# k-sheridan/ekf_vio

Hardware: AMD Instinct MI355X
Metric: filter steps/sec (predict+update) (higher is better)
Workload: dtype f32

## Files before the change

ekf_vio_amd/csrc/chol_persist.inc:

```

#ifndef PERSIST_POLL_SLEEP_LAZY
#define PERSIST_POLL_SLEEP_LAZY 12
#endif
#ifndef PERSIST_POLL_SLEEP
#define PERSIST_POLL_SLEEP 2
#endif

struct PollBound {
    int spin_limit, wait_ticks;
};
struct PersistArgs {
    float* S;
    int lds;
    float* L;
    int ldl;
    float* Linv;
    int mb, idb0;
    int* info;
    unsigned long long* Lsign;
    int* ready;
    int* fin;
    int* abort_flag;
    long long* dbg;
    PersistGrid grid;
// ... 245 lines not shown
        float yq = 0.f, rd = 0.f, ro = 0.f;
        if (sq >= 0) {
            yq = ga.zrow[cq] - ga.mu[sq];
            rd = ga.Rm[2 * cq];
            ro = ga.Rm[2 * (cq ^ 1) + 1];
        }
        tab[tid] = yq, tab[64 + tid] = rd, tab[128 + tid] = ro;
    }
    auto column_flags = [&](int kb, const int* zflag) -> PollLane {
        const int ax = alo + tid - 2;
        return {tid == 0 ? a.pan + iy * mb + kb : tid == 1 ? zflag : (tid >= 2 && ax <= ahi) ? a.pan + (mb + ax) * mb + kb : nullptr, 1};
    };
    float kv[16], w2[16];
    {
        float wv[16];
        const int scl = max(sq, 0);
#pragma unroll
        for (int ps = 0; ps < 16; ps++) wv[ps] = ga.P[(size_t)min(ib * PB + wave + 4 * ps, ga.n - 1) * ga.ld + scl];
#pragma unroll
        for (int ps = 0; ps < 16; ps++) asm volatile("" : "+v"(wv[ps]));
#pragma unroll
        for (int ps = 0; ps < 16; ps++) Th[(wave + 4 * ps) * 65 + lane] = (sq >= 0 && ib * PB + wave + 4 * ps < ga.n) ? wv[ps] : 0.f;
        __syncthreads();
#pragma unroll
        for (int q = 0; q < 16; q++) {
            kv[q] = 0.f;
            w2[q] = Th[r * 65 + mma64_col(wc, lane, q)];
        }
    }
    auto fetch = [&](int kb) -> unsigned long long {
        const bool gk = kb >= cb;
        float hv[16];
        unsigned long long neg;
        if constexpr (WAIT) {
            persist_wait(a, column_flags(kb, gk ? a.pan + iz * mb + kb : nullptr), tid, kb < mb - 2);
            load_tile_sc1(Ti, bL, (unsigned)(kb * PB) * (unsigned)ldl + (unsigned)(iy * PB), ldl, tid);
            if (gk) load_tile_sc1(Tj, bL, (unsigned)(kb * PB) * (unsigned)ldl + (unsigned)(iz * PB), ldl, tid);
#pragma unroll
            for (int ps = 0; ps < 16; ps++)
                hv[ps] = __builtin_bit_cast(float, __builtin_amdgcn_raw_buffer_load_b32(bL, ((unsigned)(kb * PB + wave + 4 * ps) * (unsigned)ldl + (unsigned)(mb * PB) + sqc) * 4u, 0, 16));
#pragma unroll
            for (int ps = 0; ps < 16; ps++) hv[ps] = (sq >= 0) ? hv[ps] : 0.f;
#pragma unroll
            for (int ps = 0; ps < 16; ps++) Th[(wave + 4 * ps) * PLD + lane] = hv[ps];
            neg = ld_sign_sc1(a.Lsign + kb);
        } else {
            load_tile(Ti, a.L + (size_t)kb * PB * ldl + (size_t)iy * PB, ldl, tid);
            if (gk) load_tile(Tj, a.L + (size_t)kb * PB * ldl + (size_t)iz * PB, ldl, tid);
#pragma unroll
            for (int ps = 0; ps < 16; ps++) hv[ps] = a.L[(size_t)(kb * PB + wave + 4 * ps) * ldl + (size_t)(mb * PB) + sqc];
#pragma unroll
            for (int ps = 0; ps < 16; ps++) hv[ps] = (sq >= 0) ? hv[ps] : 0.f;
#pragma unroll
            for (int ps = 0; ps < 16; ps++) Th[(wave + 4 * ps) * PLD + lane] = hv[ps];
            neg = a.Lsign[kb];
        }
        return neg;
    };
    auto products = [&](int kb, unsigned long long neg, bool z_unsigned) {
        if (kb >= cb) {
            const f32x16 up = (z_unsigned && neg != 0ull) ? mma64_signed(Ti, 1, PLD, Tj, 1, PLD, wr, wc, lane, neg) : mma64(Ti, 1, PLD, Tj, 1, PLD, wr, wc, lane);
#pragma unroll
            for (int q = 0; q < 16; q++) kv[q] = kv[q] + up[q];
        }
        if (alo <= ahi) {
            f32x16 up;
            if constexpr (WAIT) {
                up = (neg == 0ull) ? mma64(Ti, 1, PLD, Th, 1, PLD, wr, wc, lane) : mma64_signed(Ti, 1, PLD, Th, 1, PLD, wr, wc, lane, neg);
            } else {
                if (__builtin_amdgcn_readfirstlane((int)(neg != 0ull))) {
                    __syncthreads();
                    sign_cols(Ti, Ti, neg, tid);
                    __syncthreads();
                }
                up = mma64(Ti, 1, PLD, Th, 1, PLD, wr, wc, lane);
            }
#pragma unroll
            for (int q = 0; q < 16; q++) w2[q] = w2[q] - up[q];
        }
        if (WAIT && a.dbg && tid == 0 && mb <= 8 && (ib == 0 || ib == 6) && (cb == 0 || cb == 3 || cb == 7))
            a.dbg[100 + 8 * ((ib ? 3 : 0) + (cb == 0 ? 0 : cb == 3 ? 1 : 2)) + kb] = (long long)__builtin_amdgcn_s_memrealtime();
    };
    if constexpr (WAIT) {
        for (int kb = 0; kb < mb - 2; kb++) {
            __syncthreads();
            const unsigned long long neg = fetch(kb);
            __syncthreads();
            products(kb, neg, false);
        }
    } else {
        for (int kb = 0; kb < mb; kb++) {
            __syncthreads();
            const unsigned long long neg = fetch(kb);
            __syncthreads();
            products(kb, neg, false);
        }
    }
    if constexpr (WAIT) {
        const int kl = mb - 1, k6 = mb - 2;
        const bool gk6 = k6 >= cb;
        const __amdgpu_buffer_rsrc_t bI = persist_rsrc(a.Linv, (unsigned)(mb * PB * PB));
        const bool zi = a.grid.compact() && cb == kl;
        __syncthreads();
        persist_wait(a, column_flags(k6, gk6 ? a.pan + iz * mb + k6 : (zi ? nullptr : a.fin + iz * mb + kl)), tid, false);
        RegTile ql, qi, qj;
        float hq[16];
        unsigned long long neg6;
        {
            RegTile pi6, pj6;
            float h6[16];
            pi6.request(bL, (unsigned)(k6 * PB) * (unsigned)ldl + (unsigned)(iy * PB), ldl, tid);
            if (gk6) pj6.request(bL, (unsigned)(k6 * PB) * (unsigned)ldl + (unsigned)(iz * PB), ldl, tid);
#pragma unroll
            for (int ps = 0; ps < 16; ps++)
                h6[ps] = __builtin_bit_cast(float, __builtin_amdgcn_raw_buffer_load_b32(bL, ((unsigned)(k6 * PB + wave + 4 * ps) * (unsigned)ldl + (unsigned)(mb * PB) + sqc) * 4u, 0, 16));
            neg6 = ld_sign_sc1(a.Lsign + k6);
            pi6.put(Ti, tid);
            if (gk6) pj6.put(Tj, tid);
#pragma unroll
            for (int ps = 0; ps < 16; ps++) Th[(wave + 4 * ps) * PLD + lane] = (sq >= 0) ? h6[ps] : 0.f;
        }
        persist_wait(a, a.ready + kl, nullptr, nullptr, tid, 4, false);
        ql.request(bL, (unsigned)(kl * PB) * (unsigned)ldl + (unsigned)(kl * PB), ldl, tid);
        qi.request(bS, (unsigned)(kl * PB) * (unsigned)a.lds + (unsigned)(iy * PB), a.lds, tid);
        if (!zi) qj.request(bS, (unsigned)(kl * PB) * (unsigned)a.lds + (unsigned)(iz * PB), a.lds, tid);
        const float4 qv = ld_sc1(bI, (unsigned)(kl * PB * PB) + tid * 4);
        const unsigned long long neg7 = ld_sign_sc1(a.Lsign + kl);
#pragma unroll
        for (int ps = 0; ps < 16; ps++)
            hq[ps] = __builtin_bit_cast(float, __builtin_amdgcn_raw_buffer_load_b32(bS, ((unsigned)(kl * PB + wave + 4 * ps) * (unsigned)a.lds + (unsigned)(mb * PB) + sqc) * 4u, 0, 16));
        products(mb - 2, neg6, false);
        __syncthreads();
        ql.put(Tl, tid);
        qi.put(Ti, tid);
        if (zi) identity_tile(Tj, tid);
        else qj.put(Tj, tid);
        inv_put(qv, Tinv, tid);
#pragma unroll
        for (int ps = 0; ps < 16; ps++) Th[(wave + 4 * ps) * PLD + lane] = (sq >= 0) ? hq[ps] : 0.f;
        __syncthreads();
        float* const t3[3] = {Ti, Tj, Th};
        tri_solve_fwd_n<3>(t3, Tl, Tinv, wave, lane);
        __syncthreads();
        products(kl, neg7, true);
    }
#pragma unroll
    for (int q = 0; q < 16; q++) kv[q] = (fabsf(kv[q]) > EKF_FLUSH_THRESH) ? kv[q] : 0.f;
    float* Kt = a.K + (size_t)(cb * PB) * a.ldk + (size_t)ib * PB;
    float* Gt = ga.G + (size_t)(cb * PB) * ga.ld + (size_t)ib * PB;
    float acc = 0.f;
#pragma unroll
    for (int q = 0; q < 16; q++) {
        const int c = mma64_col(wc, lane, q), cg = cb * PB + c;
        Kt[(size_t)c * a.ldk + r] = kv[q];
        float g = 0.f;
        if (cg < m) {
            const float x = kv[q] * tab[64 + c], y = kv[q ^ 1] * tab[128 + c];
            const float kr = ((cg ^ 1) < cg) ? (y + x) : (x + y);
            g = kr - w2[q];
            acc = acc + kv[q] * tab[c];
        }
        Gt[(size_t)c * ga.ld + r] = g;
    }
    __syncthreads();
    float* part = Th;
    part[(wc * 2 + (lane >> 5)) * 64 + r] = acc;
    __syncthreads();
    if (tid < 64) ga.Wt[(size_t)cb * ga.ld + (size_t)ib * PB + tid] = ((part[tid] + part[64 + tid]) + part[128 + tid]) + part[192 + tid];
}

template <bool WAIT>
__device__ __forceinline__ void t2_tile(const PersistArgs& a, float* Ti, float* Tj, float* Tl, float* Tinv, int ta, int tb, int tid, long long* dbg = nullptr) {
    const int lane = tid & 63, wave = tid >> 6, wr = wave & 1, wc = wave >> 1;
    const int r = wr * 32 + (lane & 31);
    const int mb = a.mb, ldl = a.ldl;
    const bool diag = ta == tb;
    const __amdgpu_buffer_rsrc_t bL = persist_rsrc(a.L, (unsigned)ldl * (unsigned)(mb * PB));
    float tab[16], tba[16];
    {
        const float* sab = a.Sg + (size_t)tb * PB * a.ldsg + (size_t)ta * PB;
        const float* sba = a.Sg + (size_t)ta * PB * a.ldsg + (size_t)tb * PB;
#pragma unroll
        for (int q = 0; q < 16; q++) {
            const int c = mma64_col(wc, lane, q);
            tab[q] = sab[(size_t)c * a.ldsg + r];
            tba[q] = diag ? 0.f : sba[(size_t)c * a.ldsg + r];
        }
    }
    const int ia = mb + ta, ib = mb + tb;
    auto apply = [&](int kb, unsigned long long neg) {
        const float* Bj = diag ? Ti : Tj;
        f32x16 up;
        if constexpr (WAIT) {
            up = (neg == 0ull) ? mma64(Ti, 1, PLD, Bj, 1, PLD, wr, wc, lane) : mma64_signed(Ti, 1, PLD, Bj, 1, PLD, wr, wc, lane, neg);
        } else if (__builtin_amdgcn_readfirstlane((int)(neg != 0ull))) {
            sign_cols(Tl, Ti, neg, tid);
            __syncthreads();
            up = mma64(Tl, 1, PLD, Bj, 1, PLD, wr, wc, lane);
            __syncthreads();
        } else {
            up = mma64(Ti, 1, PLD, Bj, 1, PLD, wr, wc, lane);
        }
#pragma unroll
        for (int q = 0; q < 16; q++) tab[q] = tab[q] - up[q];
        if (!diag) {
#pragma unroll
            for (int q = 0; q < 16; q++) Tl[r * PLD + mma64_col(wc, lane, q)] = up[q];
            __syncthreads();
#pragma unroll
            for (int q = 0; q < 16; q++) tba[q] = tba[q] - Tl[mma64_col(wc, lane, q) * PLD + r];
        }
        if (dbg && tid == 0) dbg[kb] = (long long)__builtin_amdgcn_s_memrealtime();
    };
    if constexpr (WAIT) {
        for (int kb = 0; kb < mb - 2; kb++) {
            __syncthreads();
            persist_wait(a, nullptr, a.pan + ia * mb + kb, diag ? nullptr : a.pan + ib * mb + kb, tid, 1, true);
            load_tile_sc1(Ti, bL, (unsigned)(kb * PB) * (unsigned)ldl + (unsigned)(ia * PB), ldl, tid);
            if (!diag) load_tile_sc1(Tj, bL, (unsigned)(kb * PB) * (unsigned)ldl + (unsigned)(ib * PB), ldl, tid);
            const unsigned long long neg = ld_sign_sc1(a.Lsign + kb);
            __syncthreads();
            apply(kb, neg);
        }
    } else {
        for (int kb = 0; kb < mb; kb++) {
            __syncthreads();
            load_tile(Ti, a.L + (size_t)kb * PB * ldl + (size_t)ia * PB, ldl, tid);
            if (!diag) load_tile(Tj, a.L + (size_t)kb * PB * ldl + (size_t)ib * PB, ldl, tid);
            const unsigned long long neg = a.Lsign[kb];
            __syncthreads();
            apply(kb, neg);
        }
    }
    if constexpr (WAIT) {
        const int kl = mb - 1, k6 = mb - 2;
        const __amdgpu_buffer_rsrc_t bS = persist_rsrc(a.S, (unsigned)a.lds * (unsigned)(mb * PB));
        const __amdgpu_buffer_rsrc_t bI = persist_rsrc(a.Linv, (unsigned)(mb * PB * PB));
        __syncthreads();
        persist_wait(a, a.ready + kl, a.pan + ia * mb + k6, diag ? nullptr : a.pan + ib * mb + k6, tid, 4, false);
        RegTile pi6, pj6, ql, qi, qj;
        pi6.request(bL, (unsigned)(k6 * PB) * (unsigned)ldl + (unsigned)(ia * PB), ldl, tid);
        if (!diag) pj6.request(bL, (unsigned)(k6 * PB) * (unsigned)ldl + (unsigned)(ib * PB), ldl, tid);
        const unsigned long long neg6 = ld_sign_sc1(a.Lsign + k6);
        ql.request(bL, (unsigned)(kl * PB) * (unsigned)ldl + (unsigned)(kl * PB), ldl, tid);
        qi.request(bS, (unsigned)(kl * PB) * (unsigned)a.lds + (unsigned)(ia * PB), a.lds, tid);
        if (!diag) qj.request(bS, (unsigned)(kl * PB) * (unsigned)a.lds + (unsigned)(ib * PB), a.lds, tid);
        const float4 qv = ld_sc1(bI, (unsigned)(kl * PB * PB) + tid * 4);
        const unsigned long long neg7 = ld_sign_sc1(a.Lsign + kl);
        pi6.put(Ti, tid);
        if (!diag) pj6.put(Tj, tid);
        __syncthreads();
        apply(k6, neg6);
        __syncthreads();
        ql.put(Tl, tid);
        qi.put(Ti, tid);
        if (!diag) qj.put(Tj, tid);
        inv_put(qv, Tinv, tid);
        __syncthreads();
        if (diag) tri_solve_fwd(Ti, Tl, Tinv, wave, lane);
        else tri_solve_fwd2(Ti, Tj, Tl, Tinv, wave, lane);
        __syncthreads();
        apply(kl, neg7);
    }
    __syncthreads();
#pragma unroll
    for (int q = 0; q < 16; q++) {
        const int c = mma64_col(wc, lane, q);
        Ti[c * PLD + r] = (ta * PB + r < a.nstate && tb * PB + c < a.nstate) ? tab[q] : 0.f;
        if (!diag) Tj[c * PLD + r] = (tb * PB + r < a.nstate && ta * PB + c < a.nstate) ? tba[q] : 0.f;
    }
    __syncthreads();
    store_tile(Ti, a.T2 + (size_t)tb * PB * a.ldt + (size_t)ta * PB, a.ldt, tid);
    if (!diag) store_tile(Tj, a.T2 + (size_t)ta * PB * a.ldt + (size_t)tb * PB, a.ldt, tid);
    if (dbg && tid == 0) dbg[15] = (long long)__builtin_amdgcn_s_memrealtime();
}

template <bool SC1>
__device__ __forceinline__ float persist_ldf(const float* p) {
    if constexpr (SC1) return __hip_atomic_load(p, __ATOMIC_RELAXED, __HIP_MEMORY_SCOPE_AGENT);
    else return *p;
}
template <bool SC1>
__device__ __forceinline__ void persist_tile_x(f32x4 (&x)[4], const float* G, int ld, int wave, int lane) {
    const int li = lane & 15, g = lane >> 4;
#pragma unroll
    for (int b = 0; b < 4; b++)
#pragma unroll
        for (int v = 0; v < 4; v++) x[b][v] = persist_ldf<SC1>(G + (size_t)(16 * b + 4 * g + v) * ld + 16 * wave + li);
}
__device__ __forceinline__ void persist_diag_block(float* D, const float* P, int tr, int tc, int lane, unsigned long long neg) {
    const int li = lane & 15, lk = lane >> 4;
    const int rb = 16 * tr, cb = 16 * tc;
    const float* ap = P + rb + li + lk * PLD;
    const float* bp = P + cb + li + lk * PLD;
    f32x4 u = {0.f, 0.f, 0.f, 0.f};
    if (neg == 0ull) {
#pragma unroll
        for (int q = 0; q < PB; q += 4) u = __builtin_amdgcn_mfma_f32_16x16x4f32(bp[q * PLD], ap[q * PLD], u, 0, 0, 0);
    } else {
#pragma unroll 4
        for (int q = 0; q < PB; q += 4) {
            float av = ap[q * PLD];
            if ((neg >> (q + lk)) & 1ull) av = -av;
            u = __builtin_amdgcn_mfma_f32_16x16x4f32(bp[q * PLD], av, u, 0, 0, 0);
        }
    }
    float t[4];
#pragma unroll
    for (int gq = 0; gq < 4; gq++) t[gq] = D[(cb + 4 * lk + gq) * PLD + rb + li];
#pragma unroll
    for (int gq = 0; gq < 4; gq++) D[(cb + 4 * lk + gq) * PLD + rb + li] = t[gq] - u[gq];
}


struct GTile {
    int ia[16];
    int ib;
    float v[16], rd[16], ro[16];
};
__device__ __forceinline__ void gtile_idx(GTile& t, const GatherArgs& ga, int m, int rb, int cb, int mb, int idb0, int tid) {
    if (rb < mb) {
        const int c = cb * PB + (tid & 63);
        t.ib = (c < m) ? ga.idx[c] : 0;
#pragma unroll
        for (int ps = 0; ps < 16; ps++) {
            const int rc = max(min(rb * PB + (tid >> 6) + 4 * ps, m - 1), 0);
            t.ia[ps] = max(ga.idx[rc], 0);
            t.rd[ps] = ga.Rm[2 * rc];
            t.ro[ps] = ga.Rm[2 * rc + 1];
        }
    } else if (rb < idb0) {
#pragma unroll
        for (int ps = 0; ps < 16; ps++) {
            const int c = cb * PB + (tid >> 6) + 4 * ps;
            t.ia[ps] = (c < m) ? ga.idx[c] : 0;
        }
// ... 274 lines not shown
        PEXIT();
    }

    if (role.kind == ROLE_LEAD || role.kind == ROLE_LEAD_GATHER0) {
        if (!compact) gather_body<false>(ga, ga.nb1 + role.n, persist_dyn_lds);
        else if (role.kind == ROLE_LEAD_GATHER0) {
            const int cb = role.a;
            const int m = ga.m_dev ? *ga.m_dev : ga.m;
            GTile t;
            gtile_idx(t, ga, m, 1, cb, mb, a.idb0, tid);
            gtile_pin(t);
            gtile_val(t, ga, m, 1, cb, mb, a.idb0, tid);
            gtile_pinv(t);
            gtile_put(t, Tl, ga, m, 1, cb, mb, a.idb0, tid);
            __syncthreads();
            store_tile_sc1<false>(Tl, bS, (unsigned)(cb * PB) * (unsigned)lds + (unsigned)PB, lds, tid);
            persist_publish(a.fin + 1 * mb + cb, tid);
        }
        if (a.gain) {
            const int tb = role.n;
            __syncthreads();
            if (role.a < a.idb0 - mb) {
                if (a.t2) gain_tile2<true>(a, ga, Ti, Tj, Tl, Tinv, persist_dyn_lds, persist_dyn_lds + PB * PLD, role.a, role.b, tid);
                else gain_tile(a, Ti, Tj, Tl, Tinv, role.a, role.b, tid);
                if (a.dbg && tid == 0 && tb < 104) a.dbg[200 + tb] = (long long)__builtin_amdgcn_s_memrealtime();
            }
        }
        PEXIT();
    }
    const int idb0 = a.idb0;
    if (role.kind == ROLE_GATHER0) {
        const int cb = role.a;
        const int m = ga.m_dev ? *ga.m_dev : ga.m;
        GTile t;
        gtile_idx(t, ga, m, 1, cb, mb, idb0, tid);
        gtile_pin(t);
        gtile_val(t, ga, m, 1, cb, mb, idb0, tid);
        gtile_pinv(t);
        gtile_put(t, Tl, ga, m, 1, cb, mb, idb0, tid);
        __syncthreads();
        store_tile_sc1<false>(Tl, bS, (unsigned)(cb * PB) * (unsigned)lds + (unsigned)PB, lds, tid);
        persist_publish(a.fin + 1 * mb + cb, tid);
        PEXIT();
    }
    const int i = role.a, j = role.b, hidx = role.n;
    const int k0 = (i >= idb0) ? (i - idb0) : 0;
    const int klast = (i == j) ? j - 2 : j - 1;
    const unsigned oij = (unsigned)(j * PB) * (unsigned)lds + (unsigned)(i * PB);
    float tv[16];
    if (fused) {
        const int m = ga.m_dev ? *ga.m_dev : ga.m;
        const bool step0 = k0 == 0 && klast >= 0;
        GTile tn, ti_, tj_;
        gtile_idx(tn, ga, m, i, j, mb, idb0, tid);
        if (step0) {
            gtile_idx(ti_, ga, m, i, 0, mb, idb0, tid);
            if (i != j) gtile_idx(tj_, ga, m, j, 0, mb, idb0, tid);
        }
        gtile_pin(tn);
        if (step0) gtile_pin(ti_);
        gtile_val(tn, ga, m, i, j, mb, idb0, tid);
        if (step0) {
            gtile_val(ti_, ga, m, i, 0, mb, idb0, tid);
            if (i != j) gtile_val(tj_, ga, m, j, 0, mb, idb0, tid);
        }
        gtile_pinv(tn);
        gtile_put(tn, Tl, ga, m, i, j, mb, idb0, tid);
        if (step0) {
            gtile_put(ti_, Ti, ga, m, i, 0, mb, idb0, tid);
            if (i != j) gtile_put(tj_, Tj, ga, m, j, 0, mb, idb0, tid);
        }
        __syncthreads();
#pragma unroll
        for (int q = 0; q < 16; q++) tv[q] = Tl[mma64_col(wc, lane, q) * PLD + r];
        __syncthreads();
    } else {
#pragma unroll
        for (int q = 0; q < 16; q++) tv[q] = S[oij + (size_t)mma64_col(wc, lane, q) * lds + r];
    }
#define HSTAMP(n)                                                                                                       \
    do {                                                                                                                \
        if (a.dbg && i == j + 1 && i < mb && k == klast && tid == 0) a.dbg[600 + 8 * j + (n)] = (long long)__builtin_amdgcn_s_memtime(); \
    } while (0)
    unsigned long long neg = 0ull;
    int k = k0;
    for (; k <= klast; k++) {
        HSTAMP(0);
        const bool lazy = !(k == klast && i <= j + 1);
        const bool early = a.early_sources && k >= 1;
        const bool src_ident = compact && k >= 1 && i >= idb0 && i - idb0 == k;
        const int* fin_ik = src_ident ? nullptr : a.fin + i * mb + k;
        if (early) {
            persist_wait(a, nullptr, fin_ik, (i != j) ? a.fin + j * mb + k : nullptr, tid, 1, lazy);
            if (src_ident) identity_tile(Ti, tid);
            else load_tile_sc1(Ti, bS, (unsigned)(k * PB) * (unsigned)lds + (unsigned)(i * PB), lds, tid);
            if (i != j) load_tile_sc1(Tj, bS, (unsigned)(k * PB) * (unsigned)lds + (unsigned)(j * PB), lds, tid);
            persist_wait(a, a.ready + k, nullptr, nullptr, tid, 4, lazy);
        } else if (k >= 1) persist_wait(a, a.ready + k, fin_ik, (i != j) ? a.fin + j * mb + k : nullptr, tid, 4, lazy);
        else if (fused) persist_wait(a, a.ready, nullptr, nullptr, tid, 4, lazy);
        else __syncthreads();
        HSTAMP(1);
        if (k >= 1 || fused) {
            load_tile_sc1(Tl, bL, (unsigned)(k * PB) * (unsigned)ldl + (unsigned)(k * PB), ldl, tid);
            load_inv_sc1(Tinv, bI, (unsigned)(k * PB * PB), tid);
            if (k >= 1 && !early) {
                if (src_ident) identity_tile(Ti, tid);
                else load_tile_sc1(Ti, bS, (unsigned)(k * PB) * (unsigned)lds + (unsigned)(i * PB), lds, tid);
                if (i != j) load_tile_sc1(Tj, bS, (unsigned)(k * PB) * (unsigned)lds + (unsigned)(j * PB), lds, tid);
            }
            neg = ld_sign_sc1(a.Lsign + k);
        } else {
            load_tile(Tl, L, ldl, tid);
            load_inv(Tinv, a.Linv, tid);
            load_tile(Ti, S + (size_t)i * PB, lds, tid);
            if (i != j) load_tile(Tj, S + (size_t)j * PB, lds, tid);
            neg = a.Lsign[0];
        }
        __syncthreads();
        HSTAMP(2);
        if (i != j)
            tri_solve_fwd2(Ti, Tj, Tl, Tinv, wave, lane);
        else
            tri_solve_fwd(Ti, Tl, Tinv, wave, lane);
        __syncthreads();
        HSTAMP(3);
        const float* Bj = (i != j) ? Tj : Ti;
        const f32x16 up = (neg == 0ull) ? mma64(Ti, 1, PLD, Bj, 1, PLD, wr, wc, lane) : mma64_signed(Ti, 1, PLD, Bj, 1, PLD, wr, wc, lane, neg);
#pragma unroll
        for (int q = 0; q < 16; q++) tv[q] = tv[q] - up[q];
        HSTAMP(4);
    }
    k = klast;
    if (klast >= k0 || fused) {
        if (klast < k0) __syncthreads();
#pragma unroll
        for (int q = 0; q < 16; q++) Tl[mma64_col(wc, lane, q) * PLD + r] = tv[q];
        __syncthreads();
        PERSIST_TEST_DELAY(a, 0);
        store_tile_sc1<false>(Tl, bS, oij, lds, tid);
    }
    if ((int)blockIdx.x != a.stall_wg) persist_publish(a.fin + i * mb + j, tid);
    else __syncthreads();
    HSTAMP(5);
    if (a.dbg && tid == 0 && i < mb && (i == j + 1 || i == j)) a.dbg[(i == j ? 740 : 720) + j] = (long long)__builtin_amdgcn_s_memrealtime();
    if (klast >= k0 && i != j) {
        if (a.gain && i >= mb) {
            const unsigned od = (unsigned)(klast * PB) * (unsigned)ldl + (unsigned)(i * PB);
            PERSIST_TEST_DELAY(a, 1);
            if (neg != 0ull && i >= idb0) store_tile_signed_sc1(Ti, bL, od, ldl, tid, neg);
            else store_tile_sc1<false>(Ti, bL, od, ldl, tid);
            persist_publish(a.pan + i * mb + klast, tid);
        } else {
            float* dst = L + (size_t)klast * PB * ldl + (size_t)i * PB;
            if (neg != 0ull && i >= idb0) store_tile_signed(Ti, dst, ldl, tid, neg);
            else store_tile(Ti, dst, ldl, tid);
        }
    }
    if (a.t2) {
        const int p = a.grid.t2_pair_of(hidx);
        if (a.dbg && tid == 0 && hidx < 8) {
            a.dbg[192 + hidx] = (long long)__builtin_amdgcn_s_memrealtime();
        }
        if (p >= 0) {
            int ta, tb;
            t2_pair(p, ta, tb);
            long long* td = nullptr;
            const int np_ = t2_pairs(a.grid.nX);
            if (a.dbg && (p == 0 || p == np_ / 2 || p == np_ - 1)) {
                td = a.dbg + 840 + 16 * (p == 0 ? 0 : p == np_ - 1 ? 2 : 1);
                if (tid == 0) td[14] = (long long)__builtin_amdgcn_s_memrealtime();
            }
            t2_tile<true>(a, Ti, Tj, Tl, Tinv, ta, tb, tid, td);
            if (a.dbg && tid == 0 && p < 91) a.dbg[304 + p] = (long long)__builtin_amdgcn_s_memrealtime();
        }
        PEXIT();
    }
    if (j == mb - 1 && i >= mb) {
        if (i >= idb0 && i - idb0 > j) PEXIT();
        if (a.gain) PEXIT();
        persist_wait(a, a.ready + j, nullptr, nullptr, tid, 4, false);
        load_tile_sc1(Tj, bL, (unsigned)(j * PB) * (unsigned)ldl + (unsigned)(j * PB), ldl, tid);
        load_inv_sc1(Tinv, bI, (unsigned)(j * PB * PB), tid);
        const unsigned long long negl = ld_sign_sc1(a.Lsign + j);
        if (klast < k0) {
#pragma unroll
            for (int q = 0; q < 16; q++) Tl[mma64_col(wc, lane, q) * PLD + r] = tv[q];
        }
        __syncthreads();
        tri_solve_fwd(Tl, Tj, Tinv, wave, lane);
        __syncthreads();
        if (a.gain) {
            const unsigned od = (unsigned)(j * PB) * (unsigned)ldl + (unsigned)(i * PB);
            if (negl != 0ull && i >= idb0) store_tile_signed_sc1(Tl, bL, od, ldl, tid, negl);
            else store_tile_sc1<false>(Tl, bL, od, ldl, tid);
            persist_publish(a.pan + i * mb + j, tid);
        } else {
            float* dst = L + (size_t)j * PB * ldl + (size_t)i * PB;
            if (negl != 0ull && i >= idb0) store_tile_signed(Tl, dst, ldl, tid, negl);
            else store_tile(Tl, dst, ldl, tid);
        }
    }
    PEXIT();
#undef PEXIT
#undef HSTAMP
#undef PSTAMP
}

__global__ __launch_bounds__(256) void gain_tiles_kernel(PersistArgs a) {
    __shared__ __attribute__((aligned(16))) float Ti[PB * PLD];
    __shared__ __attribute__((aligned(16))) float Tj[PB * PLD];
    const int tid = threadIdx.x, lane = tid & 63, wave = tid >> 6, wr = wave & 1, wc = wave >> 1;
    const int r = wr * 32 + (lane & 31);
    const int mb = a.mb, ldl = a.ldl;
    const int ib = (int)blockIdx.x / mb, cb = (int)blockIdx.x % mb;
    const int iy = mb + ib, iz = a.idb0 + cb;
    float kv[16];
#pragma unroll
    for (int q = 0; q < 16; q++) kv[q] = 0.f;
#define GT_DECL(S) float4 ya##S##0, ya##S##1, ya##S##2, ya##S##3, za##S##0, za##S##1, za##S##2, za##S##3;
#define GT_REQ1(S, IT, KB)                                                                                                                    \
    ya##S##IT = *reinterpret_cast<const float4*>(a.L + (size_t)(KB) * PB * ldl + (size_t)iy * PB + (size_t)((tid + IT * 256) >> 4) * ldl + ((tid + IT * 256) & 15) * 4); \
    za##S##IT = *reinterpret_cast<const float4*>(a.L + (size_t)(KB) * PB * ldl + (size_t)iz * PB + (size_t)((tid + IT * 256) >> 4) * ldl + ((tid + IT * 256) & 15) * 4);
#define GT_REQ(S, KB) GT_REQ1(S, 0, KB) GT_REQ1(S, 1, KB) GT_REQ1(S, 2, KB) GT_REQ1(S, 3, KB)
#define GT_PUT1(S, IT)                                                                                        \
    *reinterpret_cast<float4*>(Ti + ((tid + IT * 256) >> 4) * PLD + ((tid + IT * 256) & 15) * 4) = ya##S##IT; \
    *reinterpret_cast<float4*>(Tj + ((tid + IT * 256) >> 4) * PLD + ((tid + IT * 256) & 15) * 4) = za##S##IT;
#define GT_STEP(S, KB)                                                      \
    do {                                                                    \
        __syncthreads();                                                    \
        GT_PUT1(S, 0) GT_PUT1(S, 1) GT_PUT1(S, 2) GT_PUT1(S, 3)             \
        __syncthreads();                                                    \
        if ((KB) + 2 < mb) { GT_REQ(S, (KB) + 2) }                          \
        const f32x16 up = mma64(Ti, 1, PLD, Tj, 1, PLD, wr, wc, lane);      \
        _Pragma("unroll") for (int q = 0; q < 16; q++) kv[q] = kv[q] + up[q]; \
    } while (0)
    GT_DECL(0)
    GT_DECL(1)
    GT_REQ(0, cb)
    if (cb + 1 < mb) { GT_REQ(1, cb + 1) }
    else { ya10 = ya11 = ya12 = ya13 = za10 = za11 = za12 = za13 = make_float4(0.f, 0.f, 0.f, 0.f); }
    for (int kb = cb; kb < mb; kb += 2) {
        GT_STEP(0, kb);
        if (kb + 1 < mb) GT_STEP(1, kb + 1);
    }
#undef GT_DECL
#undef GT_REQ1
#undef GT_REQ
#undef GT_PUT1
#undef GT_STEP
    float* Kt = a.K + (size_t)(cb * PB) * a.ldk + (size_t)ib * PB;
#pragma unroll
    for (int q = 0; q < 16; q++) {
        const int c = mma64_col(wc, lane, q);
        Kt[(size_t)c * a.ldk + r] = (fabsf(kv[q]) > EKF_FLUSH_THRESH) ? kv[q] : 0.f;
    }
}

__global__ __launch_bounds__(256) void gain2_t2_tiles_kernel(PersistArgs a, GatherArgs ga, int gain_wgs) {
    extern __shared__ float g2_dyn_lds[];
    __shared__ __attribute__((aligned(16))) float Ti[PB * PLD];
    __shared__ __attribute__((aligned(16))) float Tj[PB * PLD];
    __shared__ __attribute__((aligned(16))) float Th[PB * PLD];
    __shared__ float tab[192];
    if ((int)blockIdx.x < gain_wgs) {
        gain_tile2<false>(a, ga, Ti, Tj, nullptr, nullptr, Th, tab, (int)blockIdx.x / a.mb, (int)blockIdx.x % a.mb, threadIdx.x);
    } else {
        int ta, tb;
        t2_pair((int)blockIdx.x - gain_wgs, ta, tb);
        t2_tile<false>(a, Ti, Tj, Th, nullptr, ta, tb, threadIdx.x);
    }
}
```

ekf_vio_amd/csrc/plan.h:

```cpp
#ifndef EKFVIO_PLAN_H_
#define EKFVIO_PLAN_H_
#include <stddef.h>
#include <stdlib.h>

#include <algorithm>

#define EKF_BASE 22
#define EKF_TILE 64
#ifndef EKF_SWEEP_SPLIT_MB
#define EKF_SWEEP_SPLIT_MB 16
#endif
#define LIN_LM 8
#define GC 4
#define GCI 4

static inline int round_up(int x, int m) { return (x + m - 1) / m * m; }

struct Tuning {
    int early_status = 1;
    int upload_kernel = 1;
    int sweep_wait_ticks = 300000;
    double sweep_retry_first_s = 2.0;
    int persist_sweep = 1;
    int sweep_la = 1;
// ... 211 lines not shown
    SweepKind sweep = SWEEP_NONE;
    bool fused_gather = false;
    bool with_wt = false;
    GainBy gain = GAIN_GEMM;
    UpdateTail tail = TAIL_NONE;
    int t2_skip = -1;
    bool t2_by_sweep = false, compact = false;
    int lin_blocks = 0;
    bool persistent() const { return sweep == SWEEP_PERSIST_FUSED || sweep == SWEEP_PERSIST; }
};

enum PersistGridKind { GRID_PLAIN,
                       GRID_FUSED,
                       GRID_COMPACT };
enum PersistRoleKind { ROLE_CHAIN, ROLE_LEAD, ROLE_LEAD_GATHER0, ROLE_GATHER0, ROLE_OWNER, ROLE_NONE };
struct PersistRole {
    int kind, a, b, n;
};
PLAN_HD constexpr int t2_pairs(int nX) { return nX * (nX + 1) / 2; }
PLAN_HD void t2_pair(int p, int& ta, int& tb) {
    ta = 0;
    while ((ta + 1) * (ta + 2) / 2 <= p) ta++;
    tb = p - ta * (ta + 1) / 2;
}
struct PersistGrid {
    int kind = GRID_PLAIN;
    int mb = 0, nX = 0;
    int lead_rows = 0;
    int t2_skip = 0;
    PLAN_HD bool fused() const { return kind != GRID_PLAIN; }
    PLAN_HD bool compact() const { return kind == GRID_COMPACT; }
    PLAN_HD int lead() const { return fused() ? mb * lead_rows : 0; }
    PLAN_HD int gatherers() const { return kind == GRID_FUSED ? 2 : 0; }
    PLAN_HD int a_rows(int j) const { return mb - j - (j == 1 ? 1 : 0); }
    PLAN_HD int column_owners(int j) const { return a_rows(j) + nX + (j + 1 - (compact() ? 1 : 0)); }
    PLAN_HD int owners() const {
        int h = 0;
        for (int j = 1; j < mb; j++) h += column_owners(j);
        return h;
    }
    PLAN_HD int owner_block(int h) const { return 1 + lead() + gatherers() + h; }
    PLAN_HD int total() const { return owner_block(owners()); }
    PLAN_HD int t2_pair_of(int h) const { return (h >= t2_skip && h - t2_skip < t2_pairs(nX)) ? h - t2_skip : -1; }
    PLAN_HD PersistRole role(int block) const {
        if (block == 0) return {ROLE_CHAIN, 0, 0, 0};
        int h = block - 1;
        if (h < lead()) {
            const int ib = h / mb, cb = h % mb;
            if (compact() && cb == mb - 1 && ib < 2) return {ROLE_LEAD_GATHER0, ib, cb, h};
            return {ROLE_LEAD, ib, cb, h};
        }
        h -= lead();
        if (h < gatherers()) return {ROLE_GATHER0, h, 0, h};
        h -= gatherers();
        const int n = h;
        for (int j = 1; j < mb; j++) {
            const int nA = a_rows(j);
            if (h < column_owners(j)) {
                const int i = h < nA ? j + h + (j == 1 ? 1 : 0) : h < nA + nX ? mb + (h - nA) : mb + nX + (h - nA - nX);
                return {ROLE_OWNER, i, j, n};
            }
            h -= column_owners(j);
        }
        return {ROLE_NONE, 0, 0, n};
    }
};
#ifndef EKF_PERSIST_OVERSUB
#define EKF_PERSIST_OVERSUB 1
#endif
inline bool persist_shape(const Tuning& t, const PlanShape& s, int m_pad, int n_pad) {
    const int mb = m_pad / EKF_TILE;
    const int over = t.persist_oversub > 0 ? t.persist_oversub : EKF_PERSIST_OVERSUB;
    return mb >= 3 && mb < EKF_SWEEP_SPLIT_MB && PersistGrid{GRID_PLAIN, mb, n_pad / EKF_TILE}.total() <= (over > 1 ? over : 1) * s.num_cus &&
           persist_flag_words(m_pad, n_pad) <= s.sweep_sync_words;
}
inline bool gain_in_sweep_shape(const Tuning& t, const PlanShape& s, int m_pad, int n_pad) {
    const int mb = m_pad / EKF_TILE;
    return persist_shape(t, s, m_pad, n_pad) && PersistGrid{GRID_FUSED, mb, n_pad / EKF_TILE, s.ldp / 64}.total() <= s.num_cus + 8;
}
inline int t2_skip_owners(const Tuning& t, const PlanShape& s, int m_pad, int n_pad) {
    if (!t.t2_flow || !t.persist_gain || t.schur || !gain_in_sweep_shape(t, s, m_pad, n_pad)) return -1;
    const PersistGrid g{GRID_COMPACT, m_pad / EKF_TILE, n_pad / EKF_TILE, s.ldp / 64};
    if (g.total() > s.num_cus) return -1;
    if (g.nX + 2 > PERSIST_POLL_FLAGS) return -1;
    return (t2_pairs(g.nX) <= g.owners()) ? 0 : -1;
}
inline PersistGrid persist_grid(const UpdatePlan& p, int ldp) {
    return {p.sweep != SWEEP_PERSIST_FUSED ? GRID_PLAIN : p.compact ? GRID_COMPACT : GRID_FUSED, p.m_pad / EKF_TILE, p.n_pad / EKF_TILE, ldp / 64, p.t2_skip};
}
inline SweepKind choose_sweep(const Tuning& t, const PlanShape& s, int m_pad, int n_pad, bool filter_update) {
    const int mb = m_pad / EKF_TILE;
    const bool schur_shape = t.schur && mb < EKF_SWEEP_SPLIT_MB;
    if (schur_shape && filter_update) return SWEEP_SCHUR;
    if (t.persist_sweep && !s.latched_off && !schur_shape && s.sole_handle && persist_shape(t, s, m_pad, n_pad))
        return (filter_update && t.fuse_sweep && t.fuse_gather) ? SWEEP_PERSIST_FUSED : SWEEP_PERSIST;
    return mb < EKF_SWEEP_SPLIT_MB ? SWEEP_STEP : t.sweep_la ? SWEEP_SPLIT_LA : SWEEP_SPLIT;
}
inline bool gain_tiles_shape(const Tuning& t, const PlanShape& s, int m_pad, int n_pad) { return t.persist_gain && gain_in_sweep_shape(t, s, m_pad, n_pad); }

inline UpdatePlan plan_raw_sweep(const Tuning& t, const PlanShape& s, int m_pad, int n_pad) {
    UpdatePlan p;
    p.m = p.m_pad = m_pad, p.n_pad = n_pad;
    p.sweep = choose_sweep(t, s, m_pad, n_pad, false);
    p.gain = gain_tiles_shape(t, s, m_pad, n_pad) ? GAIN_TILES : GAIN_GEMM;
    return p;
}

inline GemmShape tail_gemm_shape(int n, int m_pad, int lin_blocks) {
    GemmShape g;
    g.M = g.N = n, g.K = m_pad, g.transB = true, g.epi = EPI_MEAN_PARTIAL, g.mean = true, g.lin_blocks = lin_blocks;
    return g;
}
inline UpdatePlan plan_update(const Tuning& t, const PlanShape& s, int m, bool m_on_device = false, float next_dt = -1.f, bool recoverable = true) {
    UpdatePlan p;
    if (m_on_device) m = 2 * s.N;
    const int n = s.n, ld = s.ldp, m_pad = round_up(m > 0 ? m : 1, EKF_TILE), n_pad = round_up(n, EKF_TILE);
    p.m = m, p.m_pad = m_pad, p.n_pad = n_pad, p.m_on_device = m_on_device, p.recoverable = recoverable;
    if (m <= 0) return p;
    p.sweep = choose_sweep(t, s, m_pad, n_pad, true);
    const bool schur = p.sweep == SWEEP_SCHUR, fused = p.sweep == SWEEP_PERSIST_FUSED;
    p.with_wt = !schur;
    if (t.fuse_gather && !fused)
        p.fused_gather = 1 + gather_element_wgs(ld, m_pad) + (schur ? 0 : (m_pad / 64) * (ld / 64)) <= s.num_cus;
    if (schur) return p.gain = GAIN_SCHUR, p.tail = TAIL_SCHUR, p;
    p.t2_skip = t2_skip_owners(t, s, m_pad, n_pad);
    if (p.t2_skip < 0) {
        p.gain = !gain_tiles_shape(t, s, m_pad, n_pad) ? GAIN_GEMM : fused ? GAIN_SWEEP : GAIN_TILES;
        return p.tail = TAIL_JOSEPH, p;
    }
    p.tail = TAIL_T2;
    p.t2_by_sweep = p.compact = fused;
    p.gain = fused ? GAIN_SWEEP : GAIN2_T2_TILES;
    const int lin_blocks = (s.N + LIN_LM - 1) / LIN_LM + 1;
    if (next_dt >= 0.f && t.lin_overlap && !s.dense_predict && t.fuse_linearize)
        p.lin_blocks = plan_gemm(t, s.num_cus, tail_gemm_shape(n, m_pad, lin_blocks)).lin_blocks;
    return p;
}

#ifndef EKF_GRAPH_STEPS
#define EKF_GRAPH_STEPS 8
#endif
#define EKF_GRAPH_STEPS_BIG 32
#define EKF_GRAPH_STEPS_PAIR 2
#define EKF_GRAPH_BIG_FROM_FRAMES (2 * EKF_GRAPH_STEPS_BIG)
#define RUN_GRAPHS 3
inline int run_graph_steps(int g) { return g == 0 ? EKF_GRAPH_STEPS_BIG : g == 1 ? EKF_GRAPH_STEPS : EKF_GRAPH_STEPS_PAIR; }
inline bool run_graph_used(int g, int frames) { return g != 0 || frames >= EKF_GRAPH_BIG_FROM_FRAMES; }
struct RunPlan {
    bool graphs = false;
    int m = 0;
    int replays[RUN_GRAPHS] = {0, 0, 0};
    int eager = 0;
};
inline int run_geometry(const int* seq_m, int i, int N, bool gated) { return gated && seq_m[i] > 0 ? 2 * N : seq_m[i]; }
inline RunPlan plan_run(const int* seq_m, int frames, int N, bool gated, bool profiling, int count) {
    RunPlan p;
    p.eager = count;
    p.graphs = !profiling && (count >= 2 || count == 0);
    for (int i = 0; p.graphs && i < frames; i++) p.graphs = run_geometry(seq_m, i, N, gated) == run_geometry(seq_m, 0, N, gated);
    if (!p.graphs) return p;
    p.m = run_geometry(seq_m, 0, N, gated);
    for (int g = 0; g < RUN_GRAPHS; g++)
        if (run_graph_used(g, frames)) p.replays[g] = p.eager / run_graph_steps(g), p.eager %= run_graph_steps(g);
    return p;
}
#endif
```

Measured before the change: 11010.

## Publish last-column panels early and fold the k6 step into main gain loops

The panel-writing workgroups now store and publish their last-column L panel inside the final k iteration, before the trailing update and the S-tile store, so downstream gain workgroups can start sooner. The gain and sweep consumers drop their special-cased k=mb-2 prefetch/apply path, run it as a normal loop iteration, and wait on a combined set of ready/fin flags for the final column. The poll-flag capacity check is tightened by one to fit the extra flag. This changes the cross-workgroup synchronisation order, which risks ordering bugs and adds extra poll lanes per workgroup.

```diff
diff --git a/ekf_vio_amd/csrc/chol_persist.inc b/ekf_vio_amd/csrc/chol_persist.inc
--- a/ekf_vio_amd/csrc/chol_persist.inc
+++ b/ekf_vio_amd/csrc/chol_persist.inc
@@ -351,7 +351,7 @@
             a.dbg[100 + 8 * ((ib ? 3 : 0) + (cb == 0 ? 0 : cb == 3 ? 1 : 2)) + kb] = (long long)__builtin_amdgcn_s_memrealtime();
     };
     if constexpr (WAIT) {
-        for (int kb = 0; kb < mb - 2; kb++) {
+        for (int kb = 0; kb < mb - 1; kb++) {
             __syncthreads();
             const unsigned long long neg = fetch(kb);
             __syncthreads();
@@ -366,30 +366,16 @@
         }
     }
     if constexpr (WAIT) {
-        const int kl = mb - 1, k6 = mb - 2;
-        const bool gk6 = k6 >= cb;
+        const int kl = mb - 1;
         const __amdgpu_buffer_rsrc_t bI = persist_rsrc(a.Linv, (unsigned)(mb * PB * PB));
         const bool zi = a.grid.compact() && cb == kl;
-        __syncthreads();
-        persist_wait(a, column_flags(k6, gk6 ? a.pan + iz * mb + k6 : (zi ? nullptr : a.fin + iz * mb + kl)), tid, false);
+        const int axl = alo + tid - 3;
+        const PollLane last_flags = {tid == 0 ? a.ready + kl : tid == 1 ? a.fin + iy * mb + kl : tid == 2 ? (zi ? nullptr : a.fin + iz * mb + kl)
+                                     : (axl <= ahi) ? a.fin + (mb + axl) * mb + kl : nullptr, tid == 0 ? 4 : 1};
+        __syncthreads();
         RegTile ql, qi, qj;
         float hq[16];
-        unsigned long long neg6;
-        {
-            RegTile pi6, pj6;
-            float h6[16];
-            pi6.request(bL, (unsigned)(k6 * PB) * (unsigned)ldl + (unsigned)(iy * PB), ldl, tid);
-            if (gk6) pj6.request(bL, (unsigned)(k6 * PB) * (unsigned)ldl + (unsigned)(iz * PB), ldl, tid);
-#pragma unroll
-            for (int ps = 0; ps < 16; ps++)
-                h6[ps] = __builtin_bit_cast(float, __builtin_amdgcn_raw_buffer_load_b32(bL, ((unsigned)(k6 * PB + wave + 4 * ps) * (unsigned)ldl + (unsigned)(mb * PB) + sqc) * 4u, 0, 16));
-            neg6 = ld_sign_sc1(a.Lsign + k6);
-            pi6.put(Ti, tid);
-            if (gk6) pj6.put(Tj, tid);
-#pragma unroll
-            for (int ps = 0; ps < 16; ps++) Th[(wave + 4 * ps) * PLD + lane] = (sq >= 0) ? h6[ps] : 0.f;
-        }
-        persist_wait(a, a.ready + kl, nullptr, nullptr, tid, 4, false);
+        persist_wait(a, last_flags, tid, false);
         ql.request(bL, (unsigned)(kl * PB) * (unsigned)ldl + (unsigned)(kl * PB), ldl, tid);
         qi.request(bS, (unsigned)(kl * PB) * (unsigned)a.lds + (unsigned)(iy * PB), a.lds, tid);
         if (!zi) qj.request(bS, (unsigned)(kl * PB) * (unsigned)a.lds + (unsigned)(iz * PB), a.lds, tid);
@@ -398,8 +384,6 @@
 #pragma unroll
         for (int ps = 0; ps < 16; ps++)
             hq[ps] = __builtin_bit_cast(float, __builtin_amdgcn_raw_buffer_load_b32(bS, ((unsigned)(kl * PB + wave + 4 * ps) * (unsigned)a.lds + (unsigned)(mb * PB) + sqc) * 4u, 0, 16));
-        products(mb - 2, neg6, false);
-        __syncthreads();
         ql.put(Tl, tid);
         qi.put(Ti, tid);
         if (zi) identity_tile(Tj, tid);
@@ -482,9 +466,9 @@
         if (dbg && tid == 0) dbg[kb] = (long long)__builtin_amdgcn_s_memrealtime();
     };
     if constexpr (WAIT) {
-        for (int kb = 0; kb < mb - 2; kb++) {
-            __syncthreads();
-            persist_wait(a, nullptr, a.pan + ia * mb + kb, diag ? nullptr : a.pan + ib * mb + kb, tid, 1, true);
+        for (int kb = 0; kb < mb - 1; kb++) {
+            __syncthreads();
+            persist_wait(a, nullptr, a.pan + ia * mb + kb, diag ? nullptr : a.pan + ib * mb + kb, tid, 1, kb < mb - 2);
             load_tile_sc1(Ti, bL, (unsigned)(kb * PB) * (unsigned)ldl + (unsigned)(ia * PB), ldl, tid);
             if (!diag) load_tile_sc1(Tj, bL, (unsigned)(kb * PB) * (unsigned)ldl + (unsigned)(ib * PB), ldl, tid);
             const unsigned long long neg = ld_sign_sc1(a.Lsign + kb);
@@ -502,25 +486,17 @@
         }
     }
     if constexpr (WAIT) {
-        const int kl = mb - 1, k6 = mb - 2;
+        const int kl = mb - 1;
         const __amdgpu_buffer_rsrc_t bS = persist_rsrc(a.S, (unsigned)a.lds * (unsigned)(mb * PB));
         const __amdgpu_buffer_rsrc_t bI = persist_rsrc(a.Linv, (unsigned)(mb * PB * PB));
         __syncthreads();
-        persist_wait(a, a.ready + kl, a.pan + ia * mb + k6, diag ? nullptr : a.pan + ib * mb + k6, tid, 4, false);
-        RegTile pi6, pj6, ql, qi, qj;
-        pi6.request(bL, (unsigned)(k6 * PB) * (unsigned)ldl + (unsigned)(ia * PB), ldl, tid);
-        if (!diag) pj6.request(bL, (unsigned)(k6 * PB) * (unsigned)ldl + (unsigned)(ib * PB), ldl, tid);
-        const unsigned long long neg6 = ld_sign_sc1(a.Lsign + k6);
+        RegTile ql, qi, qj;
+        persist_wait(a, a.ready + kl, a.fin + ia * mb + kl, diag ? nullptr : a.fin + ib * mb + kl, tid, 4, false);
         ql.request(bL, (unsigned)(kl * PB) * (unsigned)ldl + (unsigned)(kl * PB), ldl, tid);
         qi.request(bS, (unsigned)(kl * PB) * (unsigned)a.lds + (unsigned)(ia * PB), a.lds, tid);
         if (!diag) qj.request(bS, (unsigned)(kl * PB) * (unsigned)a.lds + (unsigned)(ib * PB), a.lds, tid);
         const float4 qv = ld_sc1(bI, (unsigned)(kl * PB * PB) + tid * 4);
         const unsigned long long neg7 = ld_sign_sc1(a.Lsign + kl);
-        pi6.put(Ti, tid);
-        if (!diag) pj6.put(Tj, tid);
-        __syncthreads();
-        apply(k6, neg6);
-        __syncthreads();
         ql.put(Tl, tid);
         qi.put(Ti, tid);
         if (!diag) qj.put(Tj, tid);
@@ -961,6 +937,11 @@
     do {                                                                                                                \
         if (a.dbg && i == j + 1 && i < mb && k == klast && tid == 0) a.dbg[600 + 8 * j + (n)] = (long long)__builtin_amdgcn_s_memtime(); \
     } while (0)
+#define OSTAMP(n)                                                                                                       \
+    do {                                                                                                                \
+        if (a.dbg && tid == 0 && j == mb - 1 && i >= mb && i - mb < 40) a.dbg[904 + 3 * (i - mb) + (n)] = (long long)__builtin_amdgcn_s_memrealtime(); \
+    } while (0)
+    const bool early_pan = a.gain && i >= mb && i != j;
     unsigned long long neg = 0ull;
     int k = k0;
     for (; k <= klast; k++) {
@@ -1003,37 +984,41 @@
             tri_solve_fwd(Ti, Tl, Tinv, wave, lane);
         __syncthreads();
         HSTAMP(3);
-        const float* Bj = (i != j) ? Tj : Ti;
-        const f32x16 up = (neg == 0ull) ? mma64(Ti, 1, PLD, Bj, 1, PLD, wr, wc, lane) : mma64_signed(Ti, 1, PLD, Bj, 1, PLD, wr, wc, lane, neg);
-#pragma unroll
-        for (int q = 0; q < 16; q++) tv[q] = tv[q] - up[q];
-        HSTAMP(4);
-    }
-    k = klast;
-    if (klast >= k0 || fused) {
-        if (klast < k0) __syncthreads();
-#pragma unroll
-        for (int q = 0; q < 16; q++) Tl[mma64_col(wc, lane, q) * PLD + r] = tv[q];
-        __syncthreads();
-        PERSIST_TEST_DELAY(a, 0);
-        store_tile_sc1<false>(Tl, bS, oij, lds, tid);
-    }
-    if ((int)blockIdx.x != a.stall_wg) persist_publish(a.fin + i * mb + j, tid);
-    else __syncthreads();
-    HSTAMP(5);
-    if (a.dbg && tid == 0 && i < mb && (i == j + 1 || i == j)) a.dbg[(i == j ? 740 : 720) + j] = (long long)__builtin_amdgcn_s_memrealtime();
-    if (klast >= k0 && i != j) {
-        if (a.gain && i >= mb) {
+        if (k == klast) OSTAMP(0);
+        if (early_pan && k == klast) {
             const unsigned od = (unsigned)(klast * PB) * (unsigned)ldl + (unsigned)(i * PB);
             PERSIST_TEST_DELAY(a, 1);
             if (neg != 0ull && i >= idb0) store_tile_signed_sc1(Ti, bL, od, ldl, tid, neg);
             else store_tile_sc1<false>(Ti, bL, od, ldl, tid);
-            persist_publish(a.pan + i * mb + klast, tid);
-        } else {
-            float* dst = L + (size_t)klast * PB * ldl + (size_t)i * PB;
-            if (neg != 0ull && i >= idb0) store_tile_signed(Ti, dst, ldl, tid, neg);
-            else store_tile(Ti, dst, ldl, tid);
-        }
+        }
+        const float* Bj = (i != j) ? Tj : Ti;
+        const f32x16 up = (neg == 0ull) ? mma64(Ti, 1, PLD, Bj, 1, PLD, wr, wc, lane) : mma64_signed(Ti, 1, PLD, Bj, 1, PLD, wr, wc, lane, neg);
+#pragma unroll
+        for (int q = 0; q < 16; q++) tv[q] = tv[q] - up[q];
+        HSTAMP(4);
+    }
+    k = klast;
+    if (early_pan && klast >= k0) {
+        persist_publish(a.pan + i * mb + klast, tid);
+        OSTAMP(2);
+    }
+    if (klast >= k0 || fused) {
+        if (klast < k0) __syncthreads();
+#pragma unroll
+        for (int q = 0; q < 16; q++) Tl[mma64_col(wc, lane, q) * PLD + r] = tv[q];
+        __syncthreads();
+        PERSIST_TEST_DELAY(a, 0);
+        store_tile_sc1<false>(Tl, bS, oij, lds, tid);
+    }
+    if ((int)blockIdx.x != a.stall_wg) persist_publish(a.fin + i * mb + j, tid);
+    else __syncthreads();
+    HSTAMP(5);
+    OSTAMP(1);
+    if (a.dbg && tid == 0 && i < mb && (i == j + 1 || i == j)) a.dbg[(i == j ? 740 : 720) + j] = (long long)__builtin_amdgcn_s_memrealtime();
+    if (klast >= k0 && i != j && !early_pan) {
+        float* dst = L + (size_t)klast * PB * ldl + (size_t)i * PB;
+        if (neg != 0ull && i >= idb0) store_tile_signed(Ti, dst, ldl, tid, neg);
+        else store_tile(Ti, dst, ldl, tid);
     }
     if (a.t2) {
         const int p = a.grid.t2_pair_of(hidx);
@@ -1082,6 +1067,7 @@
     PEXIT();
 #undef PEXIT
 #undef HSTAMP
+#undef OSTAMP
 #undef PSTAMP
 }
 
diff --git a/ekf_vio_amd/csrc/plan.h b/ekf_vio_amd/csrc/plan.h
--- a/ekf_vio_amd/csrc/plan.h
+++ b/ekf_vio_amd/csrc/plan.h
@@ -317,7 +317,7 @@
     if (!t.t2_flow || !t.persist_gain || t.schur || !gain_in_sweep_shape(t, s, m_pad, n_pad)) return -1;
     const PersistGrid g{GRID_COMPACT, m_pad / EKF_TILE, n_pad / EKF_TILE, s.ldp / 64};
     if (g.total() > s.num_cus) return -1;
-    if (g.nX + 2 > PERSIST_POLL_FLAGS) return -1;
+    if (g.nX + 3 > PERSIST_POLL_FLAGS) return -1;
     return (t2_pairs(g.nX) <= g.owners()) ? 0 : -1;
 }
 inline PersistGrid persist_grid(const UpdatePlan& p, int ldp) {
```

After: 11160, median of 6. 1.3% higher.
